# syshin1014/wssdl_bus

Measured on AMD Instinct MI355X. Metric: images/sec (train step, 600x1000), higher is better.
Workload: dtype f32; 1 GPU; resnet50_joint_b8; backbone=ResNet-50, image=600x1000, images_per_gpu=8, supervised_per_gpu=4, weak_per_gpu=4, mode=joint, parallelism=image-parallel dp1, RCCL grad all-reduce, sampling_rng=device, fused_rpn_softmax=True, padded_rois=False, miopen_find=True, miopen_find_db=wssdl_bus_amd/miopen_db (HIP.3_5_0_20250912-42-1199-g2584e35062), miopen_searched=True

## Files before the change

wssdl_bus_amd/csrc/plumbing/rowbn.hip:

```cpp
#include <hip/hip_runtime.h>
#include <stdint.h>

#define PLUMB_API extern "C" __attribute__((visibility("default")))

namespace {

constexpr int BLOCK = 256;
constexpr int MAX_PARTIAL_BLOCKS = 1024;

typedef float float4v __attribute__((ext_vector_type(4)));

template <int MASK>
__device__ __forceinline__ unsigned mask_roi(long long r, int div) {
    return MASK == 2 ? (unsigned)r % (unsigned)div : (unsigned)r / (unsigned)div;
}

__device__ __forceinline__ float bn_affine(float x, float sc, float sh) { return __builtin_fmaf(x, sc, sh); }
__device__ __forceinline__ float bn_dx(float ka, float u, float k0, float k1, float x) {
    return __builtin_fmaf(-k1, x, __builtin_fmaf(ka, u, -k0));
}
__device__ __forceinline__ void acc_rows2(double &s, double &q, float v0, float w0, float v1, float w1) {
    s += (double)v0 + (double)v1;
    q += (double)v0 * (double)w0 + (double)v1 * (double)w1;
}
// ... 4 lines not shown

struct Slab {
    int C4, L, RS, lc, lr;
    long long r0, r1;
    __device__ __forceinline__ Slab(long long M, int C, long long rows_per_block) {
        C4 = C >> 2;
        L = C4 < BLOCK ? C4 : BLOCK;
        RS = BLOCK / L;
        lc = threadIdx.x % L;
        lr = threadIdx.x / L;
        r0 = (long long)blockIdx.x * rows_per_block;
        r1 = r0 + rows_per_block < M ? r0 + rows_per_block : M;
    }
};

__device__ __forceinline__ void slab_reduce(const Slab &b, int C, int c4, const double (&s)[4], const double (&q)[4],
                                            double (*red)[8], double *__restrict__ out) {
    const int t = threadIdx.x;
    __syncthreads();
#pragma unroll
    for (int j = 0; j < 4; ++j) { red[t][j] = s[j]; red[t][4 + j] = q[j]; }
    __syncthreads();
    if (b.lr == 0) {
#pragma unroll
        for (int j = 0; j < 4; ++j) {
            double ss = 0.0, qq = 0.0;
            for (int k = 0; k < b.RS; ++k) { ss += red[k * b.L + b.lc][j]; qq += red[k * b.L + b.lc][4 + j]; }
            out[c4 * 4 + j] = ss;
            out[C + c4 * 4 + j] = qq;
        }
    }
}

template <int MODE, bool RELU, int MASK>
__global__ __launch_bounds__(BLOCK) void rowbn_partial_kernel(
    const float *__restrict__ x, const float *__restrict__ dy, const float *__restrict__ scale,
    const float *__restrict__ shift, long long M, int C, long long rows_per_block,
    double *__restrict__ partial, const float *__restrict__ mask, int per) {
    __shared__ double red[BLOCK][8];
    const Slab b(M, C, rows_per_block);
    const int C4 = b.C4, L = b.L, RS = b.RS, lc = b.lc, lr = b.lr;
    const long long r0 = b.r0, r1 = b.r1;
    double *out = partial + (size_t)blockIdx.x * 2 * C;
    for (int cc = 0; cc * L < C4; ++cc) {
        const int c4 = cc * L + lc;
        double s[4] = {0, 0, 0, 0}, q[4] = {0, 0, 0, 0};
        float4v sc = {0, 0, 0, 0}, sh = {0, 0, 0, 0};
        if (MODE == 1 && RELU) {
            sc = reinterpret_cast<const float4v *>(scale)[c4];
            sh = reinterpret_cast<const float4v *>(shift)[c4];
        }
        if (lr < RS) {
            long long r = r0 + lr;
            for (; r + RS < r1; r += 2 * RS) {
                bool live0 = true, live1 = true;
                if (MASK) {
                    live0 = mask[mask_roi<MASK>(r, per)] != 0.0f;
                    live1 = mask[mask_roi<MASK>(r + RS, per)] != 0.0f;
                    if (!live0 && !live1) continue;
                }
                const float4v zero4 = {0, 0, 0, 0};
                const float4v a0 = live0 ? reinterpret_cast<const float4v *>(x + (size_t)r * C)[c4] : zero4;
                const float4v a1 = live1 ? reinterpret_cast<const float4v *>(x + (size_t)(r + RS) * C)[c4] : zero4;
                float4v g0, g1;
                if (MODE == 1) {
                    g0 = live0 ? reinterpret_cast<const float4v *>(dy + (size_t)r * C)[c4] : zero4;
                    g1 = live1 ? reinterpret_cast<const float4v *>(dy + (size_t)(r + RS) * C)[c4] : zero4;
                }
#pragma unroll
                for (int j = 0; j < 4; ++j) {
                    if (MODE == 0) {
                        acc_rows2(s[j], q[j], a0[j], a0[j], a1[j], a1[j]);
                    } else {
                        float u0 = g0[j], u1 = g1[j];
                        if (RELU) {
                            if (!(bn_affine(a0[j], sc[j], sh[j]) > 0.0f)) u0 = 0.0f;
                            if (!(bn_affine(a1[j], sc[j], sh[j]) > 0.0f)) u1 = 0.0f;
                        }
                        if (MASK) {
                            if (!live0) u0 = 0.0f;
                            if (!live1) u1 = 0.0f;
                        }
                        acc_rows2(s[j], q[j], u0, a0[j], u1, a1[j]);
                    }
                }
            }
            for (; r < r1; r += RS) {
                if (MASK && mask[mask_roi<MASK>(r, per)] == 0.0f) continue;
                const float4v a0 = reinterpret_cast<const float4v *>(x + (size_t)r * C)[c4];
                float4v g0;
                if (MODE == 1) g0 = reinterpret_cast<const float4v *>(dy + (size_t)r * C)[c4];
#pragma unroll
                for (int j = 0; j < 4; ++j) {
                    if (MODE == 0) {
                        acc_row(s[j], q[j], a0[j], a0[j]);
                    } else {
                        float u0 = g0[j];
                        if (RELU && !(bn_affine(a0[j], sc[j], sh[j]) > 0.0f)) u0 = 0.0f;
                        acc_row(s[j], q[j], u0, a0[j]);
                    }
                }
            }
        }
        slab_reduce(b, C, c4, s, q, red, out);
    }
}

constexpr int FIN_COLS = 16, FIN_GROUPS = 64;

__device__ __forceinline__ void finish_reduce(const double *__restrict__ partial, int nblocks, int C,
                                              int c, int grp, double (*red)[FIN_COLS][2], double &s,
                                              double &q) {
    double ss = 0.0, qq = 0.0;
    if (c < C)
        for (int b = grp; b < nblocks; b += FIN_GROUPS) {
            ss += partial[(size_t)b * 2 * C + c];
            qq += partial[(size_t)b * 2 * C + C + c];
        }
    red[grp][threadIdx.x % FIN_COLS][0] = ss;
    red[grp][threadIdx.x % FIN_COLS][1] = qq;
    __syncthreads();
    s = 0.0;
    q = 0.0;
    if (grp == 0)
// ... 64 lines not shown
    dweight[c] = (float)sum_g_xhat;
    dbias[c] = (float)sg;
    coef[c] = (float)a;
    coef[C + c] = (float)k0;
    coef[2 * C + c] = (float)k1;
}

template <bool RELU, int MASK>
__global__ __launch_bounds__(BLOCK) void rowbn_apply_fwd_kernel(
    const float *__restrict__ x, const float *__restrict__ scale, const float *__restrict__ shift,
    long long total4, int C4, float *__restrict__ y, const float *__restrict__ mask, int per) {
    for (long long i = (long long)blockIdx.x * BLOCK + threadIdx.x; i < total4;
         i += (long long)gridDim.x * BLOCK) {
        const int c4 = (int)(i % C4);
        if (MASK && mask[mask_roi<MASK>(i / C4, per)] == 0.0f) {
            const float4v zero4 = {0, 0, 0, 0};
            reinterpret_cast<float4v *>(y)[i] = zero4;
            continue;
        }
        const float4v a = reinterpret_cast<const float4v *>(x)[i];
        const float4v sc = reinterpret_cast<const float4v *>(scale)[c4];
        const float4v sh = reinterpret_cast<const float4v *>(shift)[c4];
        float4v o;
#pragma unroll
        for (int j = 0; j < 4; ++j) {
            float v = bn_affine(a[j], sc[j], sh[j]);
            if (RELU) v = v > 0.0f ? v : 0.0f;
            o[j] = v;
        }
        reinterpret_cast<float4v *>(y)[i] = o;
    }
}

template <bool RELU, int MASK>
__global__ __launch_bounds__(BLOCK) void rowbn_apply_bwd_kernel(
    const float *__restrict__ x, const float *__restrict__ dy, const float *__restrict__ scale,
    const float *__restrict__ shift, const float *__restrict__ coef, long long total4, int C4,
    float *__restrict__ dx, const float *__restrict__ mask, int per) {
    const int C = C4 * 4;
    for (long long i = (long long)blockIdx.x * BLOCK + threadIdx.x; i < total4;
         i += (long long)gridDim.x * BLOCK) {
        const int c4 = (int)(i % C4);
        if (MASK && mask[mask_roi<MASK>(i / C4, per)] == 0.0f) {
            const float4v zero4 = {0, 0, 0, 0};
            reinterpret_cast<float4v *>(dx)[i] = zero4;
            continue;
        }
        const float4v a = reinterpret_cast<const float4v *>(x)[i];
        const float4v g = reinterpret_cast<const float4v *>(dy)[i];
        const float4v ka = reinterpret_cast<const float4v *>(coef)[c4];
        const float4v k0 = reinterpret_cast<const float4v *>(coef + C)[c4];
        const float4v k1 = reinterpret_cast<const float4v *>(coef + 2 * C)[c4];
        float4v sc = {0, 0, 0, 0}, sh = {0, 0, 0, 0};
        if (RELU) {
            sc = reinterpret_cast<const float4v *>(scale)[c4];
            sh = reinterpret_cast<const float4v *>(shift)[c4];
        }
        float4v o;
#pragma unroll
        for (int j = 0; j < 4; ++j) {
            float u = g[j];
            if (RELU && !(bn_affine(a[j], sc[j], sh[j]) > 0.0f)) u = 0.0f;
            o[j] = bn_dx(ka[j], u, k0[j], k1[j], a[j]);
        }
        reinterpret_cast<float4v *>(dx)[i] = o;
    }
}


template <int MASK>
__device__ __forceinline__ bool row_live(const float *__restrict__ mask, long long r, int div) {
    return MASK ? mask[mask_roi<MASK>(r, div)] != 0.0f : true;
}

__device__ __forceinline__ float4v load4(const float *__restrict__ p, long long r, int C, int c4, bool on) {
    const float4v zero4 = {0, 0, 0, 0};
    return on ? reinterpret_cast<const float4v *>(p + (size_t)r * C)[c4] : zero4;
}

template <bool DUAL, int MASK>
__global__ __launch_bounds__(BLOCK) void rowbn_join_fwd_kernel(
    const float *__restrict__ x3, const float *__restrict__ sc3, const float *__restrict__ sh3,
// ... 286 lines not shown
                         workspace, workspace_bytes, stream);
}

PLUMB_API int wsplumb_rowbn_backward_masked(const float *x, const float *dy, long long M, int C,
                                            const float *weight, const float *mean, const float *rstd,
                                            const float *scale, const float *shift, int relu,
                                            const float *mask, int n_rois, int per, float *dx,
                                            float *dweight, float *dbias, float *coef, void *workspace,
                                            size_t workspace_bytes, void *stream) {
    if (!mask) return 1;
    return backward_impl(x, dy, M, C, weight, mean, rstd, scale, shift, relu, dx, dweight, dbias, coef, mask, n_rois, per,
                         workspace, workspace_bytes, stream);
}

PLUMB_API int wsplumb_rowbn_forward_masked_pm(const float *x, long long M, int C, const float *weight,
                                              const float *bias, float eps, int relu, const float *mask,
                                              int n_rois, int per, float *y, float *mean, float *var,
                                              float *rstd, float *scale, float *shift, float *count,
                                              void *workspace, size_t workspace_bytes, void *stream) {
    if (!mask || !count) return 1;
    return forward_impl(x, M, C, weight, bias, eps, relu, y, mean, var, rstd, scale, shift, mask, n_rois, per, count,
                        workspace, workspace_bytes, stream, true);
}

PLUMB_API int wsplumb_rowbn_backward_masked_pm(const float *x, const float *dy, long long M, int C,
                                               const float *weight, const float *mean, const float *rstd,
                                               const float *scale, const float *shift, int relu,
                                               const float *mask, int n_rois, int per, float *dx,
                                               float *dweight, float *dbias, float *coef, void *workspace,
                                               size_t workspace_bytes, void *stream) {
    if (!mask) return 1;
    return backward_impl(x, dy, M, C, weight, mean, rstd, scale, shift, relu, dx, dweight, dbias, coef, mask, n_rois, per,
                         workspace, workspace_bytes, stream, true);
}


PLUMB_API size_t wsplumb_rowbn_join_workspace_bytes(long long M, int C) {
    return 2 * wsplumb_rowbn_workspace_bytes(M, C);
}

namespace {

struct JoinGeom {
    hipStream_t st;
    int nb, mode, div;
    long long rpb, total4;
    double *p0, *p1;
};

inline int join_geom(long long M, int C, const float *mask, int n_rois, int per, void *workspace,
                     size_t workspace_bytes, void *stream, JoinGeom &g) {
    if (!shape_ok(M, C) || workspace_bytes < wsplumb_rowbn_join_workspace_bytes(M, C)) return 1;
    if (mask && (per < 1 || n_rois < 1 || (long long)n_rois * per != M || M > 0x7fffffffLL)) return 1;
    g.st = static_cast<hipStream_t>(stream);
    g.nb = partial_blocks(M, C);
    g.rpb = (M + g.nb - 1) / g.nb;
    g.total4 = M * (C / 4);
    g.mode = mask ? 2 : 0;
    g.div = mask ? n_rois : 1;
    g.p0 = static_cast<double *>(workspace);
    g.p1 = g.p0 + (size_t)g.nb * 2 * C;
    return 0;
}

inline void join_stats(const JoinGeom &g, const float *x, long long M, int C, const float *weight, const float *bias,
                       float eps, float *stats, const float *mask, int n_rois, int per, float *count) {
// ... 99 lines not shown
```

wssdl_bus_amd/csrc/plumbing/taps.hip:

```cpp
#include <hip/hip_runtime.h>
#include <stdint.h>

#define PLUMB_API extern "C" __attribute__((visibility("default")))

namespace {

constexpr int TAB_NCLS = 0, TAB_H = 1, TAB_W = 2, TAB_OH = 3, TAB_OW = 4, TAB_S = 5, TAB_PT = 6, TAB_PL = 7,
              TAB_UNITS = 8, TAB_WUNITS = 9;
constexpr int TAB_CLS = 16, CLS_STRIDE = 24, MAX_CLS = 9;
constexpr int C_NPOS = 0, C_NTAPS = 1, C_SLOT = 2, C_CUM = 3, C_WCUM = 4,
              C_TAPS = 6,
              C_TAPIDX = 15;
constexpr int MAX_POS = 64;
constexpr int TAB_SLOTPOS = TAB_CLS + CLS_STRIDE * MAX_CLS;
constexpr int TAB_POSSLOT = TAB_SLOTPOS + MAX_POS;
constexpr int TAB_SLOTCLS = TAB_POSSLOT + MAX_POS;
constexpr int TAB_INTS = TAB_SLOTCLS + MAX_POS;

typedef float float4v __attribute__((ext_vector_type(4)));

__device__ __forceinline__ const int *cls_of(const int *T, int k) { return T + TAB_CLS + CLS_STRIDE * k; }

template <int F>
__device__ __forceinline__ int find_class(const int *__restrict__ T, unsigned q) {
    const int n = T[TAB_NCLS];
    int k = 0;
    while (k + 1 < n && (unsigned)cls_of(T, k + 1)[F] <= q) ++k;
    return k;
}

__global__ __launch_bounds__(256) void tap_gather_kernel(const float *__restrict__ x, const int *__restrict__ T,
                                                        int in_pm, unsigned R, unsigned C4, unsigned total4,
                                                        float *__restrict__ cols) {
    const int H = T[TAB_H], W = T[TAB_W], OW = T[TAB_OW], S = T[TAB_S], PT = T[TAB_PT], PL = T[TAB_PL];
    const unsigned unit4 = R * C4;
    for (unsigned i = blockIdx.x * 256u + threadIdx.x; i < total4; i += gridDim.x * 256u) {
        const int k = find_class<C_CUM>(T, i / unit4);
        const int *cl = cls_of(T, k);
        const unsigned ntaps = cl[C_NTAPS];
        const unsigned local = i - (unsigned)cl[C_CUM] * unit4;
        const unsigned c4 = local % C4, t = local / C4;
        const unsigned tl = t % ntaps, row = t / ntaps;
        const unsigned roi = row % R, p = row / R;
        const int pos = T[TAB_SLOTPOS + cl[C_SLOT] + p];
        const int tap = cl[C_TAPS + tl];
        const int y = (pos / OW) * S + tap / 3 - PT, xx = (pos % OW) * S + tap % 3 - PL;
        float4v v = {0.f, 0.f, 0.f, 0.f};
        if (y >= 0 && y < H && xx >= 0 && xx < W) {
            const size_t src = in_pm ? (size_t)T[TAB_POSSLOT + y * W + xx] * R + roi
                                     : ((size_t)roi * H + y) * W + xx;
            v = reinterpret_cast<const float4v *>(x)[src * C4 + c4];
        }
        reinterpret_cast<float4v *>(cols)[i] = v;
    }
}

__global__ __launch_bounds__(256) void tap_col2im_kernel(const float *__restrict__ dcols, const int *__restrict__ T,
                                                        int in_pm, unsigned R, unsigned C4, unsigned total4,
                                                        float *__restrict__ dx) {
    const int H = T[TAB_H], W = T[TAB_W], OH = T[TAB_OH], OW = T[TAB_OW], S = T[TAB_S], PT = T[TAB_PT],
              PL = T[TAB_PL];
    const unsigned unit4 = R * C4;
    for (unsigned i = blockIdx.x * 256u + threadIdx.x; i < total4; i += gridDim.x * 256u) {
        const unsigned c4 = i % C4, row = i / C4;
        unsigned roi;
        int y, xx;
        if (in_pm) {
            roi = row % R;
            const int pos = T[TAB_SLOTPOS + row / R];
            y = pos / W;
            xx = pos % W;
        } else {
            xx = (int)(row % (unsigned)W);
            const unsigned t = row / (unsigned)W;
            y = (int)(t % (unsigned)H);
            roi = t / (unsigned)H;
        }
        float4v acc = {0.f, 0.f, 0.f, 0.f};
#pragma unroll
        for (int ky = 0; ky < 3; ++ky) {
            const int ny = y + PT - ky;
            if (ny < 0 || ny % S != 0) continue;
            const int oy = ny / S;
            if (oy >= OH) continue;
#pragma unroll
            for (int kx = 0; kx < 3; ++kx) {
                const int nx = xx + PL - kx;
                if (nx < 0 || nx % S != 0) continue;
                const int ox = nx / S;
                if (ox >= OW) continue;
                const int slot = T[TAB_POSSLOT + oy * OW + ox];
                const int *cl = cls_of(T, T[TAB_SLOTCLS + slot]);
                const int tl = cl[C_TAPIDX + ky * 3 + kx];
                if (tl < 0) continue;
                const size_t u = (size_t)cl[C_CUM] * unit4 +
                                 (((size_t)(slot - cl[C_SLOT]) * R + roi) * cl[C_NTAPS] + tl) * C4 + c4;
                acc += reinterpret_cast<const float4v *>(dcols)[u];
            }
        }
        reinterpret_cast<float4v *>(dx)[i] = acc;
    }
}

__global__ __launch_bounds__(256) void tap_weight_gather_kernel(const float *__restrict__ w, const int *__restrict__ T,
                                                               unsigned CO, unsigned C4, unsigned total4,
                                                               float *__restrict__ wp) {
    const unsigned unit4 = CO * C4;
    for (unsigned i = blockIdx.x * 256u + threadIdx.x; i < total4; i += gridDim.x * 256u) {
        const int k = find_class<C_WCUM>(T, i / unit4);
        const int *cl = cls_of(T, k);
        const unsigned ntaps = cl[C_NTAPS];
        const unsigned local = i - (unsigned)cl[C_WCUM] * unit4;
        const unsigned c4 = local % C4, t = local / C4;
        const unsigned tl = t % ntaps, o = t / ntaps;
        reinterpret_cast<float4v *>(wp)[i] =
            reinterpret_cast<const float4v *>(w)[((size_t)o * 9 + cl[C_TAPS + tl]) * C4 + c4];
    }
}

__global__ __launch_bounds__(256) void tap_weight_scatter_kernel(const float *__restrict__ dwp, const int *__restrict__ T,
                                                                unsigned CO, unsigned C4, unsigned total4,
                                                                float *__restrict__ dw) {
    const int n = T[TAB_NCLS];
    const unsigned unit4 = CO * C4;
    for (unsigned i = blockIdx.x * 256u + threadIdx.x; i < total4; i += gridDim.x * 256u) {
        const unsigned c4 = i % C4, t = i / C4;
        const unsigned tap = t % 9u, o = t / 9u;
        float4v acc = {0.f, 0.f, 0.f, 0.f};
        for (int k = 0; k < n; ++k) {
            const int *cl = cls_of(T, k);
            const int tl = cl[C_TAPIDX + tap];
            if (tl < 0) continue;
            acc += reinterpret_cast<const float4v *>(dwp)[(size_t)cl[C_WCUM] * unit4 +
                                                           ((size_t)o * cl[C_NTAPS] + tl) * C4 + c4];
        }
        reinterpret_cast<float4v *>(dw)[i] = acc;
    }
}

inline int grid_for(unsigned total4) {
    unsigned b = (total4 + 255u) / 256u;
    return (int)(b < 262144u ? b : 262144u);
}

inline bool dims_ok(long long R, int C, long long total4) {
    return R >= 1 && C >= 4 && !(C & 3) && total4 >= 1 && total4 <= 0x7fffffffLL;
}

}

PLUMB_API int wsplumb_tap_table_ints() { return TAB_INTS; }

PLUMB_API int wsplumb_tap_gather(const float *x, long long R, int C, const int *tab, const int *hnum, int in_pm,
                                 float *cols, void *stream) {
    const long long total4 = (long long)hnum[TAB_UNITS] * R * (C / 4);
    if (R < 1 || C < 4 || (C & 3)) return 1;
    if (!dims_ok(R, C, total4) || (long long)hnum[TAB_H] * hnum[TAB_W] * R * (C / 4) > 0x7fffffffLL) return 2;
    hipLaunchKernelGGL(tap_gather_kernel, dim3(grid_for((unsigned)total4)), dim3(256), 0,
                       static_cast<hipStream_t>(stream), x, tab, in_pm, (unsigned)R, (unsigned)(C / 4),
                       (unsigned)total4, cols);
    return hipGetLastError() == hipSuccess ? 0 : 3;
}

PLUMB_API int wsplumb_tap_col2im(const float *dcols, long long R, int C, const int *tab, const int *hnum, int in_pm,
                                 float *dx, void *stream) {
    const long long total4 = (long long)hnum[TAB_H] * hnum[TAB_W] * R * (C / 4);
    if (R < 1 || C < 4 || (C & 3)) return 1;
    if (!dims_ok(R, C, total4) || (long long)hnum[TAB_UNITS] * R * (C / 4) > 0x7fffffffLL) return 2;
    hipLaunchKernelGGL(tap_col2im_kernel, dim3(grid_for((unsigned)total4)), dim3(256), 0,
                       static_cast<hipStream_t>(stream), dcols, tab, in_pm, (unsigned)R, (unsigned)(C / 4),
                       (unsigned)total4, dx);
    return hipGetLastError() == hipSuccess ? 0 : 3;
}

PLUMB_API int wsplumb_tap_weight_gather(const float *w, int CO, int C, const int *tab, const int *hnum, float *wp,
                                        void *stream) {
    const long long total4 = (long long)hnum[TAB_WUNITS] * CO * (C / 4);
    if (CO < 1 || !dims_ok(CO, C, total4) || 9LL * CO * (C / 4) > 0x7fffffffLL) return 1;
    hipLaunchKernelGGL(tap_weight_gather_kernel, dim3(grid_for((unsigned)total4)), dim3(256), 0,
                       static_cast<hipStream_t>(stream), w, tab, (unsigned)CO, (unsigned)(C / 4), (unsigned)total4, wp);
    return hipGetLastError() == hipSuccess ? 0 : 3;
}

PLUMB_API int wsplumb_tap_weight_scatter(const float *dwp, int CO, int C, const int *tab, const int *hnum, float *dw,
                                         void *stream) {
    const long long total4 = 9LL * CO * (C / 4);
    if (CO < 1 || !dims_ok(CO, C, total4) || (long long)hnum[TAB_WUNITS] * CO * (C / 4) > 0x7fffffffLL) return 1;
    hipLaunchKernelGGL(tap_weight_scatter_kernel, dim3(grid_for((unsigned)total4)), dim3(256), 0,
                       static_cast<hipStream_t>(stream), dwp, tab, (unsigned)CO, (unsigned)(C / 4), (unsigned)total4, dw);
    return hipGetLastError() == hipSuccess ? 0 : 3;
}
```

wssdl_bus_amd/networks/_plumbing.py:

```python
import ctypes
import os
import warnings

import torch

_HERE = os.path.dirname(os.path.dirname(os.path.abspath(__file__)))
LIB_PATH = os.path.join(_HERE, "libwssdl_plumbing_hip.so")
_lib = None
_warned = [False]

_vp, _i, _ll, _f, _sz = ctypes.c_void_p, ctypes.c_int, ctypes.c_longlong, ctypes.c_float, ctypes.c_size_t


def lib():
    global _lib
    if _lib is None:
        if not os.path.exists(LIB_PATH):
            if not _warned[0]:
                _warned[0] = True
                warnings.warn("%s not built: the per-RoI head uses stock PyTorch batch-norm ops "
                              "(python -m wssdl_bus_amd.build builds it)" % LIB_PATH)
            return None
        L = ctypes.CDLL(LIB_PATH)
        L.wsplumb_rowbn_workspace_bytes.restype = _sz
        L.wsplumb_rowbn_workspace_bytes.argtypes = [_ll, _i]
        L.wsplumb_rowbn_supported.restype = _i
        L.wsplumb_rowbn_supported.argtypes = [_ll, _i]
        L.wsplumb_rowbn_forward.restype = _i
        L.wsplumb_rowbn_forward.argtypes = [_vp, _ll, _i, _vp, _vp, _f, _i, _vp, _vp, _vp, _vp, _vp, _vp,
                                            _vp, _sz, _vp]
        L.wsplumb_rowbn_apply.restype = _i
        L.wsplumb_rowbn_apply.argtypes = [_vp, _ll, _i, _vp, _vp, _i, _vp, _vp]
        L.wsplumb_rowbn_backward.restype = _i
        L.wsplumb_rowbn_backward.argtypes = [_vp, _vp, _ll, _i, _vp, _vp, _vp, _vp, _vp, _i, _vp, _vp, _vp,
                                             _vp, _vp, _sz, _vp]
        L.wsplumb_rowbn_forward_masked.restype = _i
        L.wsplumb_rowbn_forward_masked.argtypes = [_vp, _ll, _i, _vp, _vp, _f, _i, _vp, _i, _i, _vp, _vp, _vp, _vp,
                                                   _vp, _vp, _vp, _vp, _sz, _vp]
        L.wsplumb_rowbn_backward_masked.restype = _i
        L.wsplumb_rowbn_backward_masked.argtypes = [_vp, _vp, _ll, _i, _vp, _vp, _vp, _vp, _vp, _i, _vp, _i, _i,
                                                    _vp, _vp, _vp, _vp, _vp, _sz, _vp]
        for name in ("wsplumb_rowbn_forward_masked_pm", "wsplumb_rowbn_backward_masked_pm"):
            base = getattr(L, name[:-3])
            getattr(L, name).restype, getattr(L, name).argtypes = base.restype, base.argtypes
        L.wsplumb_rowbn_join_workspace_bytes.restype = _sz
        L.wsplumb_rowbn_join_workspace_bytes.argtypes = [_ll, _i]
        L.wsplumb_rowbn_join_forward.restype = _i
        L.wsplumb_rowbn_join_forward.argtypes = [_vp, _vp, _ll, _i, _vp, _vp, _f, _vp, _vp, _f, _vp, _vp, _f, _vp, _i, _i,
                                                 _vp, _vp, _vp, _vp, _vp, _vp, _vp, _sz, _vp]
        L.wsplumb_rowbn_join_backward.restype = _i
        L.wsplumb_rowbn_join_backward.argtypes = [_vp] * 5 + [_ll, _i] + [_vp] * 7 + [_i, _i] + [_vp] * 8 + [_sz, _vp]
        L.wsplumb_tap_table_ints.restype = _i
        L.wsplumb_tap_table_ints.argtypes = []
        for name in ("wsplumb_tap_gather", "wsplumb_tap_col2im"):
            f = getattr(L, name)
            f.restype = _i
            f.argtypes = [_vp, _ll, _i, _vp, _vp, _i, _vp, _vp]
        for name in ("wsplumb_tap_weight_gather", "wsplumb_tap_weight_scatter"):
            f = getattr(L, name)
            f.restype = _i
            f.argtypes = [_vp, _i, _i, _vp, _vp, _vp, _vp]
        for name in ("wsplumb_im2col3x3", "wsplumb_col2im3x3"):
            f = getattr(L, name)
            f.restype = _i
            f.argtypes = [_vp, _ll, _i, _i, _i, _i, _i, _i, _i, _i, _vp, _vp]
        _lib = L
    return _lib


def _p(t):
    return ctypes.c_void_p(t.data_ptr())


def _stream():
    return ctypes.c_void_p(torch.cuda.current_stream().cuda_stream)


# ... 38 lines not shown


def rowbn_apply(x, scale, shift, relu):
    L = lib()
    M, C = x.shape
    y = torch.empty_like(x)
    with torch.cuda.device(x.device):
        rc = L.wsplumb_rowbn_apply(_p(x), M, C, _p(scale), _p(shift), int(relu), _p(y), _stream())
    if rc:
        raise RuntimeError("wsplumb_rowbn_apply failed (%d)" % rc)
    return y


def rowbn_backward(x, dy, weight, stats, relu, mask=None, pos_major=False):
    L = lib()
    M, C = x.shape
    dev = x.device
    dx = torch.empty_like(x)
    dwb = torch.empty((2, C), dtype=torch.float32, device=dev)
    coef = torch.empty((3, C), dtype=torch.float32, device=dev)
    with torch.cuda.device(dev):
        ws, n = _workspace(L, M, C, dev)
        if mask is None:
            rc = L.wsplumb_rowbn_backward(_p(x), _p(dy), M, C, _p(weight), _p(stats[0]), _p(stats[2]),
                                          _p(stats[3]), _p(stats[4]), int(relu), _p(dx), _p(dwb[0]),
                                          _p(dwb[1]), _p(coef), _p(ws), n, _stream())
        else:
            n_rois = mask.shape[0]
            fn = L.wsplumb_rowbn_backward_masked_pm if pos_major else L.wsplumb_rowbn_backward_masked
            rc = fn(_p(x), _p(dy), M, C, _p(weight), _p(stats[0]), _p(stats[2]), _p(stats[3]), _p(stats[4]), int(relu),
                    _p(mask), n_rois, M // n_rois, _p(dx), _p(dwb[0]), _p(dwb[1]), _p(coef), _p(ws), n, _stream())
    if rc:
        raise RuntimeError("wsplumb_rowbn_backward failed (%d)" % rc)
    return dx, dwb[0], dwb[1]


def join_usable(x):
    if os.environ.get("WSSDL_HEAD_UNFUSED_JOIN"):
        return False
    return usable(x)


def _pn(t):
    return _p(t) if t is not None else None


def rowbn_join_forward(x3, bn3, other, bns, bnn, mask=None):
    L = lib()
    M, C = x3.shape
    dev = x3.device
    assert other.shape == x3.shape and other.is_contiguous() and other.dtype == torch.float32
    out, y = torch.empty_like(x3), torch.empty_like(x3)
    stats = torch.empty((3, 5, C), dtype=torch.float32, device=dev)
    count, n_rois = None, 0
    if mask is not None:
        n_rois = mask.shape[0]
        assert M % n_rois == 0 and mask.dtype == torch.float32 and mask.is_contiguous()
        count = torch.empty((1,), dtype=torch.float32, device=dev)
    ws_, bs_, es_ = bns if bns is not None else (None, None, 0.0)
    with torch.cuda.device(dev):
        n = L.wsplumb_rowbn_join_workspace_bytes(M, C)
        ws = torch.empty((n,), dtype=torch.uint8, device=dev)
        rc = L.wsplumb_rowbn_join_forward(_p(x3), _p(other), M, C, _p(bn3[0]), _p(bn3[1]), float(bn3[2]), _pn(ws_),
                                          _pn(bs_), float(es_), _p(bnn[0]), _p(bnn[1]), float(bnn[2]), _pn(mask), n_rois,
                                          M // n_rois if n_rois else 1, _p(out), _p(y), _p(stats[0]),
                                          _p(stats[1]) if bns is not None else None, _p(stats[2]), _pn(count), _p(ws), n,
# ... 115 lines not shown
    def _table(self):
        import numpy as np
        T = np.full(_TAB_INTS, -1, np.int32)
        T[:10] = [len(self.classes), self.h, self.w, self.oh, self.ow, self.s, self.pt, self.pl, self.units,
                  self.wunits]
        for k, (taps, pos) in enumerate(self.classes[:_MAX_CLS]):
            b = _TAB_CLS + _CLS_STRIDE * k
            T[b:b + 5] = [len(pos), len(taps), self.slot_base[k], self.cum[k], self.wcum[k]]
            T[b + 6:b + 6 + len(taps)] = taps
            for i, t in enumerate(taps):
                T[b + 15 + t] = i
        for sl, (y, x) in enumerate(self.slots[:_MAX_POS]):
            T[_TAB_SLOTPOS + sl] = y * self.ow + x
            T[_TAB_POSSLOT + y * self.ow + x] = sl
            T[_TAB_SLOTCLS + sl] = next(k for k in range(len(self.classes))
                                        if self.slot_base[k] <= sl < self.slot_base[k] + len(self.classes[k][1]))
        return T

    def device_table(self, dev):
        t = self._dev.get(dev)
        if t is None:
            t = self._dev[dev] = torch.from_numpy(self.table).to(dev)
        return t

    def subsample_index(self, w_in, s, dev):
        key = ("sub", w_in, s, dev)
        t = self._dev.get(key)
        if t is None:
            t = self._dev[key] = torch.tensor([y * s * w_in + x * s for y, x in self.slots],
                                              dtype=torch.long, device=dev)
        return t


_PLANS = {}


def tap_plan(h, w, s):
    p = _PLANS.get((h, w, s))
    if p is None:
        p = _PLANS[(h, w, s)] = TapPlan(h, w, s)
    return p


def taps_usable(x):
    if os.environ.get("WSSDL_HEAD_DENSE_3X3"):
        return False
    return im2col_usable(x) and x.shape[0] >= TAPS_MIN_ROIS


def _tap_call(name, *args):
    rc = getattr(lib(), name)(*args, _stream())
    if rc:
        raise RuntimeError("%s failed (%d)" % (name, rc))


def tap_gather(x, plan, in_pm, R):
    C = x.shape[-1]
    cols = torch.empty((plan.units * R * C,), dtype=torch.float32, device=x.device)
    with torch.cuda.device(x.device):
        _tap_call("wsplumb_tap_gather", _p(x), R, C, _p(plan.device_table(x.device)), plan.hnum, int(in_pm), _p(cols))
    return cols


def tap_col2im(dcols, plan, in_pm, R, C):
    shape = (plan.h * plan.w * R, C) if in_pm else (R, plan.h, plan.w, C)
    dx = torch.empty(shape, dtype=torch.float32, device=dcols.device)
# ... 95 lines not shown
```

wssdl_bus_amd/networks/roi_head.py:

```python
import torch
import torch.nn as nn
import torch.nn.functional as F

from . import _plumbing
from .backbones import RESNET_DEFS, _same_pad


class _RowBatchNormFn(torch.autograd.Function):

    @staticmethod
    def forward(ctx, x, weight, bias, eps):
        var, mean = torch.var_mean(x, dim=0, unbiased=False)
        rstd = torch.rsqrt(var + eps)
        scale = rstd * weight
        y = torch.addcmul(bias - mean * scale, x, scale)
        ctx.save_for_backward(x, mean, rstd, weight)
        ctx.mark_non_differentiable(mean, var)
        return y, mean, var

    @staticmethod
    def backward(ctx, dy, _dmean, _dvar):
        x, mean, rstd, weight = ctx.saved_tensors
        m = x.shape[0]
        sum_dy = dy.sum(0)
# ... 29 lines not shown
            x, weight, stats, roi_mask = ctx.saved_tensors
        else:
            (x, weight, stats), roi_mask = ctx.saved_tensors, None
        dx, dw, db = _plumbing.rowbn_backward(x, dy.contiguous(), weight, stats, ctx.relu, roi_mask, ctx.pos_major)
        return dx, dw, db, None, None, None, None


class _JoinFn(torch.autograd.Function):

    @staticmethod
    def forward(ctx, x3, other, w3, b3, ws, bs, wn, bn, eps3, eps_s, eps_n, roi_mask):
        dual = ws is not None
        out, y, st3, sts, stn, count = _plumbing.rowbn_join_forward(
            x3, (w3, b3, eps3), other, (ws, bs, eps_s) if dual else None, (wn, bn, eps_n), roi_mask)
        ctx.dual, ctx.masked = dual, roi_mask is not None
        ctx.save_for_backward(x3, other if dual else None, out, w3, ws, wn, st3, sts, stn, roi_mask)
        if count is None:
            count = stn[0, :1]
        ctx.mark_non_differentiable(st3, sts, stn, count)
        ctx.set_materialize_grads(False)
        return out, y, st3, sts, stn, count

    @staticmethod
    def backward(ctx, dres, dy, *_):
        x3, xs, out, w3, ws, wn, st3, sts, stn, roi_mask = ctx.saved_tensors
        if dy is None:
            dy = torch.zeros_like(out)
        g, dx3, dxs, dwbn, dwb3, dwbs = _plumbing.rowbn_join_backward(
            out, dy.contiguous(), dres.contiguous() if dres is not None else None, x3, xs, wn, stn, w3, st3, ws, sts,
            roi_mask)
        if ctx.dual:
            return dx3, dxs, dwb3[0], dwb3[1], dwbs[0], dwbs[1], dwbn[0], dwbn[1], None, None, None, None
        return dx3, g, dwb3[0], dwb3[1], None, None, dwbn[0], dwbn[1], None, None, None, None


_ROI_MASK = None


def set_roi_mask(mask):
    global _ROI_MASK
    _ROI_MASK = mask


def _masked_row_batch_norm(x, weight, bias, eps, relu, roi_mask, pos_major=False):
    M = x.shape[0]
    per = M // roi_mask.shape[0]
    m = (roi_mask.repeat(per) if pos_major else roi_mask.repeat_interleave(per)).unsqueeze(1)
    n = (roi_mask.sum() * per).clamp_min(1.0)
    mean = (x * m).sum(0) / n
    d = (x - mean) * m
    var = (d * d).sum(0) / n
    y = d * (torch.rsqrt(var + eps) * weight) + bias
    if relu:
        y = F.relu(y)
    return y * m, mean.detach(), var.detach(), n


class RowBatchNorm(nn.Module):

    def __init__(self, num_features, eps=1e-3, momentum=0.01):
        super().__init__()
        self.eps, self.momentum = eps, momentum
        self.weight = nn.Parameter(torch.ones(num_features))
        self.bias = nn.Parameter(torch.zeros(num_features))
        self.register_buffer("running_mean", torch.zeros(num_features))
        self.register_buffer("running_var", torch.ones(num_features))
# ... 86 lines not shown
    return x.view(r, h * w, c).transpose(0, 1).index_select(0, idx).reshape(-1, c)


def _bn_rows(bn, x, relu=False):
    r, h, w, c = x.shape
    return bn(x.reshape(-1, c), relu=relu).view(r, h, w, c)


class BottleneckNHWC(nn.Module):
    expansion = 4

    def __init__(self, c_i, c_o, s, preact, norm):
        super().__init__()
        self.preact = preact
        self.pre_bn = RowBatchNorm(c_i) if (preact != "no_preact" and norm == "BN") else None
        self.conv1 = ConvNHWC(c_i, c_o, 1, 1, norm)
        self.conv2 = ConvNHWC(c_o, c_o, 3, s, norm)
        self.conv3 = ConvNHWC(c_o, c_o * 4, 1, 1, norm, relu=False)
        self.short = ConvNHWC(c_i, c_o * 4, 1, s, norm, relu=False) if c_i != c_o * 4 else None

    def forward(self, x):
        ori = x
        if self.preact != "no_preact":
            y = _bn_rows(self.pre_bn, x, relu=True) if self.pre_bn is not None else F.relu(x)
            if self.preact == "both_preact":
                ori = y
            x = y
        x = self.conv3(self.conv2(self.conv1(x)))
        return x + (self.short(ori) if self.short is not None else ori)

    def forward_pm(self, x, plans, R, pre=None, nxt=None):
        pm = x.dim() == 2
        ori = x
        if self.preact != "no_preact":
            y = pre if pre is not None else _pre_act(self.pre_bn, x, pm)
            if self.preact == "both_preact":
                ori = y
            x = y
        s = self.conv2.s
        plan = plans[s]
        if not pm:
            x = self.conv1(x)
        else:
            x = self.conv1.forward_pm(x, plan, R)
        x = self.conv3.forward_pm(self.conv2.forward_pm(x, plan, R), plan, R, act=False)
        return _join_pm(self.conv3, x, self.short, ori, plan, s, R, nxt)


class BasicBlockNHWC(nn.Module):
    expansion = 1

    def __init__(self, c_i, c_o, s, preact, norm):
        super().__init__()
        self.preact = preact
        self.pre_bn = RowBatchNorm(c_i) if (preact != "no_preact" and norm == "BN") else None
        self.conv1 = ConvNHWC(c_i, c_o, 3, s, norm)
        self.conv2 = ConvNHWC(c_o, c_o, 3, 1, norm, relu=False)
        self.short = ConvNHWC(c_i, c_o, 1, s, norm, relu=False) if c_i != c_o else None

    def forward(self, x):
        ori = x
        if self.preact != "no_preact":
            y = _bn_rows(self.pre_bn, x, relu=True) if self.pre_bn is not None else F.relu(x)
            if self.preact == "both_preact":
                ori = y
            x = y
        x = self.conv2(self.conv1(x))
        return x + (self.short(ori) if self.short is not None else ori)

    def forward_pm(self, x, plans, R, pre=None, nxt=None):
        pm = x.dim() == 2
        ori = x
        if self.preact != "no_preact":
            y = pre if pre is not None else _pre_act(self.pre_bn, x, pm)
            if self.preact == "both_preact":
                ori = y
            x = y
        s = self.conv1.s
        plan = plans[s]
        x = self.conv2.forward_pm(self.conv1.forward_pm(x, plan, R), plans[1], R, act=False)
        return _join_pm(self.conv2, x, self.short, ori, plan, s, R, nxt)


def _join_pm(last, x3, short, ori, plan, s, R, nxt):
    if short is not None:
        xs = short.forward_pm(ori, plan, R, act=False)
    else:
        xs = ori if ori.dim() == 2 else _pm_rows(ori, plan, s)
    bns = [last.bn, nxt] + ([short.bn] if short is not None else [])
    mask = _ROI_MASK
    if (nxt is None or any(b is None or not b.training for b in bns) or last.relu or not _plumbing.join_usable(x3)
            or (mask is not None and x3.shape[0] % mask.shape[0] != 0)):
        return last._act(x3, pos_major=True) + (short._act(xs, pos_major=True) if short is not None else xs), None
    b3, bs = last.bn, short.bn if short is not None else None
    out, y, st3, sts, stn, n = _JoinFn.apply(
        x3, xs.contiguous(), b3.weight, b3.bias, bs.weight if bs is not None else None,
        bs.bias if bs is not None else None, nxt.weight, nxt.bias, b3.eps, bs.eps if bs is not None else 0.0, nxt.eps,
        mask)
    n = n[0] if mask is not None else x3.shape[0]
    b3._track(st3[0], st3[1], n)
    if bs is not None:
        bs._track(sts[0], sts[1], n)
    nxt._track(stn[0], stn[1], n)
    return out, y


def _pre_act(bn, x, pm):
    if not pm:
        return _bn_rows(bn, x, relu=True) if bn is not None else F.relu(x)
    return bn(x, relu=True, pos_major=True) if bn is not None else F.relu(x)


class ResNetHeadNHWC(nn.Module):

    def __init__(self, depth, norm="BN"):
        super().__init__()
        defs, block = RESNET_DEFS[depth]
        blk = BottleneckNHWC if block.expansion == 4 else BasicBlockNHWC
        e = blk.expansion
        blocks = [blk(256 * e, 512, 2, "both_preact", norm)]
        for _ in range(1, defs[3]):
            blocks.append(blk(512 * e, 512, 1, "default", norm))
        self.group3 = nn.Sequential(*blocks)
        self.norm = RowBatchNorm(512 * e) if norm == "BN" else None
        self.out_features = 512 * e

    def forward(self, x):
        plans = self._tap_plans(x)
        if plans is not None:
            return self._forward_pm(x, plans)
        x = self.group3(x)
        x = _bn_rows(self.norm, x, relu=True) if self.norm is not None else F.relu(x)
        return x.mean(dim=(1, 2))

    @staticmethod
    def _tap_plans(x):
        if not _plumbing.taps_usable(x):
            return None
        p2 = _plumbing.tap_plan(x.shape[1], x.shape[2], 2)
# ... 16 lines not shown
```

Measured before the change: 52.78 images/s.

## Fuse head entry BN backward with shortcut grad scatter; restructure tap gather/col2im grids

Adds a fused entry path for the first ROI-head bottleneck: the pre-activation BN forward also produces the subsampled position-major rows for the shortcut, and its backward folds the shortcut gradient (scattered through a position-to-slot table) into the BN backward kernels. This removes a separate scatter/add and extra passes over the gradient. Separately, the tap gather and col2im kernels are rewritten to use a 2D grid (ROI chunks by tap unit or position), hoisting table lookups and address math per block and coalescing channel loads. The extra indirect load per dy element and the new grid limits are the main risks.

```diff
diff --git a/wssdl_bus_amd/csrc/plumbing/rowbn.hip b/wssdl_bus_amd/csrc/plumbing/rowbn.hip
--- a/wssdl_bus_amd/csrc/plumbing/rowbn.hip
+++ b/wssdl_bus_amd/csrc/plumbing/rowbn.hip
@@ -60,11 +60,29 @@
     }
 }
 
-template <int MODE, bool RELU, int MASK>
+struct EntryGrad {
+    const float *dys;
+    const int *possel;
+    int per, R;
+};
+
+template <bool ENTRY>
+__device__ __forceinline__ float4v load_dy(const float *__restrict__ dy, const EntryGrad &e, long long r, int C, int c4) {
+    const float4v g = reinterpret_cast<const float4v *>(dy + (size_t)r * C)[c4];
+    if (!ENTRY) return g;
+    const unsigned roi = (unsigned)r / (unsigned)e.per, p = (unsigned)r - roi * (unsigned)e.per;
+    const int slot = e.possel[p];
+    const float4v zero4 = {0, 0, 0, 0};
+    float4v d = zero4;
+    if (slot >= 0) d = reinterpret_cast<const float4v *>(e.dys + ((size_t)slot * e.R + roi) * C)[c4] + zero4;
+    return g + d;
+}
+
+template <int MODE, bool RELU, int MASK, bool ENTRY = false>
 __global__ __launch_bounds__(BLOCK) void rowbn_partial_kernel(
     const float *__restrict__ x, const float *__restrict__ dy, const float *__restrict__ scale,
     const float *__restrict__ shift, long long M, int C, long long rows_per_block,
-    double *__restrict__ partial, const float *__restrict__ mask, int per) {
+    double *__restrict__ partial, const float *__restrict__ mask, int per, EntryGrad eg = EntryGrad()) {
     __shared__ double red[BLOCK][8];
     const Slab b(M, C, rows_per_block);
     const int C4 = b.C4, L = b.L, RS = b.RS, lc = b.lc, lr = b.lr;
@@ -92,8 +110,8 @@
                 const float4v a1 = live1 ? reinterpret_cast<const float4v *>(x + (size_t)(r + RS) * C)[c4] : zero4;
                 float4v g0, g1;
                 if (MODE == 1) {
-                    g0 = live0 ? reinterpret_cast<const float4v *>(dy + (size_t)r * C)[c4] : zero4;
-                    g1 = live1 ? reinterpret_cast<const float4v *>(dy + (size_t)(r + RS) * C)[c4] : zero4;
+                    g0 = live0 ? load_dy<ENTRY>(dy, eg, r, C, c4) : zero4;
+                    g1 = live1 ? load_dy<ENTRY>(dy, eg, r + RS, C, c4) : zero4;
                 }
 #pragma unroll
                 for (int j = 0; j < 4; ++j) {
@@ -117,7 +135,7 @@
                 if (MASK && mask[mask_roi<MASK>(r, per)] == 0.0f) continue;
                 const float4v a0 = reinterpret_cast<const float4v *>(x + (size_t)r * C)[c4];
                 float4v g0;
-                if (MODE == 1) g0 = reinterpret_cast<const float4v *>(dy + (size_t)r * C)[c4];
+                if (MODE == 1) g0 = load_dy<ENTRY>(dy, eg, r, C, c4);
 #pragma unroll
                 for (int j = 0; j < 4; ++j) {
                     if (MODE == 0) {
@@ -248,11 +266,11 @@
     }
 }
 
-template <bool RELU, int MASK>
+template <bool RELU, int MASK, bool ENTRY = false>
 __global__ __launch_bounds__(BLOCK) void rowbn_apply_bwd_kernel(
     const float *__restrict__ x, const float *__restrict__ dy, const float *__restrict__ scale,
     const float *__restrict__ shift, const float *__restrict__ coef, long long total4, int C4,
-    float *__restrict__ dx, const float *__restrict__ mask, int per) {
+    float *__restrict__ dx, const float *__restrict__ mask, int per, EntryGrad eg = EntryGrad()) {
     const int C = C4 * 4;
     for (long long i = (long long)blockIdx.x * BLOCK + threadIdx.x; i < total4;
          i += (long long)gridDim.x * BLOCK) {
@@ -263,7 +281,7 @@
             continue;
         }
         const float4v a = reinterpret_cast<const float4v *>(x)[i];
-        const float4v g = reinterpret_cast<const float4v *>(dy)[i];
+        const float4v g = ENTRY ? load_dy<true>(dy, eg, i / C4, C, c4) : reinterpret_cast<const float4v *>(dy)[i];
         const float4v ka = reinterpret_cast<const float4v *>(coef)[c4];
         const float4v k0 = reinterpret_cast<const float4v *>(coef + C)[c4];
         const float4v k1 = reinterpret_cast<const float4v *>(coef + 2 * C)[c4];
@@ -616,6 +634,39 @@
     if (!mask) return 1;
     return backward_impl(x, dy, M, C, weight, mean, rstd, scale, shift, relu, dx, dweight, dbias, coef, mask, n_rois, per,
                          workspace, workspace_bytes, stream, true);
+}
+
+PLUMB_API int wsplumb_rowbn_backward_entry(const float *x, const float *dy, const float *dys, const int *possel,
+                                           int n_slots, long long M, int C, const float *weight, const float *mean,
+                                           const float *rstd, const float *scale, const float *shift,
+                                           const float *mask, int n_rois, int per, float *dx, float *dweight,
+                                           float *dbias, float *coef, void *workspace, size_t workspace_bytes,
+                                           void *stream) {
+    if (!shape_ok(M, C) || workspace_bytes < wsplumb_rowbn_workspace_bytes(M, C)) return 1;
+    if (!dys || !possel || per < 1 || n_rois < 1 || n_slots < 1 || n_slots > per ||
+        (long long)n_rois * per != M || M > 0x7fffffffLL)
+        return 1;
+    hipStream_t st = static_cast<hipStream_t>(stream);
+    const int nb = partial_blocks(M, C);
+    const long long rpb = (M + nb - 1) / nb;
+    double *partial = static_cast<double *>(workspace);
+    const EntryGrad eg = {dys, possel, per, n_rois};
+    if (mask)
+        hipLaunchKernelGGL((rowbn_partial_kernel<1, true, 1, true>), dim3(nb), dim3(BLOCK), 0, st, x, dy, scale, shift, M,
+                           C, rpb, partial, mask, per, eg);
+    else
+        hipLaunchKernelGGL((rowbn_partial_kernel<1, true, 0, true>), dim3(nb), dim3(BLOCK), 0, st, x, dy, scale, shift, M,
+                           C, rpb, partial, mask, 1, eg);
+    hipLaunchKernelGGL(rowbn_bwd_finish_kernel, dim3((C + FIN_COLS - 1) / FIN_COLS), dim3(FIN_COLS * FIN_GROUPS), 0, st,
+                       partial, nb, C, M, weight, mean, rstd, dweight, dbias, coef, mask, n_rois, per);
+    const long long total4 = M * (C / 4);
+    if (mask)
+        hipLaunchKernelGGL((rowbn_apply_bwd_kernel<true, 1, true>), dim3(apply_grid(total4)), dim3(BLOCK), 0, st, x, dy,
+                           scale, shift, coef, total4, C / 4, dx, mask, per, eg);
+    else
+        hipLaunchKernelGGL((rowbn_apply_bwd_kernel<true, 0, true>), dim3(apply_grid(total4)), dim3(BLOCK), 0, st, x, dy,
+                           scale, shift, coef, total4, C / 4, dx, mask, 1, eg);
+    return hipGetLastError() == hipSuccess ? 0 : 3;
 }
 
 
diff --git a/wssdl_bus_amd/csrc/plumbing/taps.hip b/wssdl_bus_amd/csrc/plumbing/taps.hip
--- a/wssdl_bus_amd/csrc/plumbing/taps.hip
+++ b/wssdl_bus_amd/csrc/plumbing/taps.hip
@@ -29,76 +29,93 @@
     return k;
 }
 
+struct RoiWalk {
+    unsigned L, RS, lc, lr, roi0, roi1;
+    __device__ __forceinline__ RoiWalk(unsigned R, unsigned C4, unsigned chunk) {
+        L = (C4 <= 256u && 256u % C4 == 0u) ? C4 : 256u;
+        RS = 256u / L;
+        lc = threadIdx.x % L;
+        lr = threadIdx.x / L;
+        roi0 = blockIdx.x * chunk;
+        roi1 = roi0 + chunk < R ? roi0 + chunk : R;
+    }
+};
+
+constexpr unsigned GATHER_CHUNK = 32, COL2IM_CHUNK = 16;
+
 __global__ __launch_bounds__(256) void tap_gather_kernel(const float *__restrict__ x, const int *__restrict__ T,
-                                                        int in_pm, unsigned R, unsigned C4, unsigned total4,
+                                                        int in_pm, unsigned R, unsigned C4,
                                                         float *__restrict__ cols) {
     const int H = T[TAB_H], W = T[TAB_W], OW = T[TAB_OW], S = T[TAB_S], PT = T[TAB_PT], PL = T[TAB_PL];
-    const unsigned unit4 = R * C4;
-    for (unsigned i = blockIdx.x * 256u + threadIdx.x; i < total4; i += gridDim.x * 256u) {
-        const int k = find_class<C_CUM>(T, i / unit4);
-        const int *cl = cls_of(T, k);
-        const unsigned ntaps = cl[C_NTAPS];
-        const unsigned local = i - (unsigned)cl[C_CUM] * unit4;
-        const unsigned c4 = local % C4, t = local / C4;
-        const unsigned tl = t % ntaps, row = t / ntaps;
-        const unsigned roi = row % R, p = row / R;
-        const int pos = T[TAB_SLOTPOS + cl[C_SLOT] + p];
-        const int tap = cl[C_TAPS + tl];
-        const int y = (pos / OW) * S + tap / 3 - PT, xx = (pos % OW) * S + tap % 3 - PL;
-        float4v v = {0.f, 0.f, 0.f, 0.f};
-        if (y >= 0 && y < H && xx >= 0 && xx < W) {
-            const size_t src = in_pm ? (size_t)T[TAB_POSSLOT + y * W + xx] * R + roi
-                                     : ((size_t)roi * H + y) * W + xx;
-            v = reinterpret_cast<const float4v *>(x)[src * C4 + c4];
-        }
-        reinterpret_cast<float4v *>(cols)[i] = v;
+    const unsigned q = blockIdx.y;
+    const int *cl = cls_of(T, find_class<C_CUM>(T, q));
+    const unsigned ntaps = cl[C_NTAPS], local = q - (unsigned)cl[C_CUM];
+    const unsigned p = local / ntaps, tl = local - p * ntaps;
+    const int pos = T[TAB_SLOTPOS + cl[C_SLOT] + p];
+    const int tap = cl[C_TAPS + tl];
+    const int y = (pos / OW) * S + tap / 3 - PT, xx = (pos % OW) * S + tap % 3 - PL;
+    const bool inside = y >= 0 && y < H && xx >= 0 && xx < W;
+    const unsigned sbase = !inside ? 0u : in_pm ? (unsigned)T[TAB_POSSLOT + y * W + xx] * R * C4 : (unsigned)(y * W + xx) * C4;
+    const unsigned sstride = in_pm ? C4 : (unsigned)(H * W) * C4;
+    const unsigned dstride = ntaps * C4;
+    const unsigned dbase = (unsigned)cl[C_CUM] * R * C4 + p * R * dstride + tl * C4;
+    const float4v *__restrict__ src = reinterpret_cast<const float4v *>(x) + sbase;
+    float4v *__restrict__ dst = reinterpret_cast<float4v *>(cols) + dbase;
+    const RoiWalk w(R, C4, GATHER_CHUNK);
+    const float4v zero4 = {0.f, 0.f, 0.f, 0.f};
+    for (unsigned c4 = w.lc; c4 < C4; c4 += w.L) {
+        unsigned roi = w.roi0 + w.lr;
+        for (; roi + 3u * w.RS < w.roi1; roi += 4u * w.RS) {
+            float4v v[4];
+#pragma unroll
+            for (int k = 0; k < 4; ++k) v[k] = inside ? src[(roi + k * w.RS) * sstride + c4] : zero4;
+#pragma unroll
+            for (int k = 0; k < 4; ++k) dst[(roi + k * w.RS) * dstride + c4] = v[k];
+        }
+        for (; roi < w.roi1; roi += w.RS) dst[roi * dstride + c4] = inside ? src[roi * sstride + c4] : zero4;
     }
 }
 
 __global__ __launch_bounds__(256) void tap_col2im_kernel(const float *__restrict__ dcols, const int *__restrict__ T,
-                                                        int in_pm, unsigned R, unsigned C4, unsigned total4,
+                                                        int in_pm, unsigned R, unsigned C4,
                                                         float *__restrict__ dx) {
     const int H = T[TAB_H], W = T[TAB_W], OH = T[TAB_OH], OW = T[TAB_OW], S = T[TAB_S], PT = T[TAB_PT],
               PL = T[TAB_PL];
-    const unsigned unit4 = R * C4;
-    for (unsigned i = blockIdx.x * 256u + threadIdx.x; i < total4; i += gridDim.x * 256u) {
-        const unsigned c4 = i % C4, row = i / C4;
-        unsigned roi;
-        int y, xx;
-        if (in_pm) {
-            roi = row % R;
-            const int pos = T[TAB_SLOTPOS + row / R];
-            y = pos / W;
-            xx = pos % W;
-        } else {
-            xx = (int)(row % (unsigned)W);
-            const unsigned t = row / (unsigned)W;
-            y = (int)(t % (unsigned)H);
-            roi = t / (unsigned)H;
-        }
-        float4v acc = {0.f, 0.f, 0.f, 0.f};
-#pragma unroll
-        for (int ky = 0; ky < 3; ++ky) {
-            const int ny = y + PT - ky;
-            if (ny < 0 || ny % S != 0) continue;
-            const int oy = ny / S;
-            if (oy >= OH) continue;
-#pragma unroll
-            for (int kx = 0; kx < 3; ++kx) {
-                const int nx = xx + PL - kx;
-                if (nx < 0 || nx % S != 0) continue;
-                const int ox = nx / S;
-                if (ox >= OW) continue;
-                const int slot = T[TAB_POSSLOT + oy * OW + ox];
-                const int *cl = cls_of(T, T[TAB_SLOTCLS + slot]);
-                const int tl = cl[C_TAPIDX + ky * 3 + kx];
-                if (tl < 0) continue;
-                const size_t u = (size_t)cl[C_CUM] * unit4 +
-                                 (((size_t)(slot - cl[C_SLOT]) * R + roi) * cl[C_NTAPS] + tl) * C4 + c4;
-                acc += reinterpret_cast<const float4v *>(dcols)[u];
-            }
-        }
-        reinterpret_cast<float4v *>(dx)[i] = acc;
+    const int pos = in_pm ? T[TAB_SLOTPOS + blockIdx.y] : (int)blockIdx.y;
+    const int y = pos / W, xx = pos % W;
+    unsigned base[9], stride[9], valid = 0;
+#pragma unroll
+    for (int ky = 0; ky < 3; ++ky) {
+#pragma unroll
+        for (int kx = 0; kx < 3; ++kx) {
+            const int j = ky * 3 + kx;
+            base[j] = stride[j] = 0;
+            const int ny = y + PT - ky, nx = xx + PL - kx;
+            if (ny < 0 || ny % S != 0 || nx < 0 || nx % S != 0) continue;
+            const int oy = ny / S, ox = nx / S;
+            if (oy >= OH || ox >= OW) continue;
+            const int slot = T[TAB_POSSLOT + oy * OW + ox];
+            const int *cl = cls_of(T, T[TAB_SLOTCLS + slot]);
+            const int tl = cl[C_TAPIDX + j];
+            if (tl < 0) continue;
+            stride[j] = (unsigned)cl[C_NTAPS] * C4;
+            base[j] = (unsigned)cl[C_CUM] * R * C4 + (unsigned)(slot - cl[C_SLOT]) * R * stride[j] + (unsigned)tl * C4;
+            valid |= 1u << j;
+        }
+    }
+    const float4v *__restrict__ src = reinterpret_cast<const float4v *>(dcols);
+    const unsigned dbase = in_pm ? blockIdx.y * R * C4 : (unsigned)pos * C4;
+    const unsigned dstride = in_pm ? C4 : (unsigned)(H * W) * C4;
+    float4v *__restrict__ dst = reinterpret_cast<float4v *>(dx) + dbase;
+    const RoiWalk w(R, C4, COL2IM_CHUNK);
+    for (unsigned c4 = w.lc; c4 < C4; c4 += w.L) {
+        for (unsigned roi = w.roi0 + w.lr; roi < w.roi1; roi += w.RS) {
+            float4v acc = {0.f, 0.f, 0.f, 0.f};
+#pragma unroll
+            for (int j = 0; j < 9; ++j)
+                if (valid & (1u << j)) acc += src[base[j] + roi * stride[j] + c4];
+            dst[roi * dstride + c4] = acc;
+        }
     }
 }
 
@@ -143,6 +160,8 @@
     return (int)(b < 262144u ? b : 262144u);
 }
 
+inline unsigned roi_chunks(long long R, unsigned chunk) { return (unsigned)((R + chunk - 1) / chunk); }
+
 inline bool dims_ok(long long R, int C, long long total4) {
     return R >= 1 && C >= 4 && !(C & 3) && total4 >= 1 && total4 <= 0x7fffffffLL;
 }
@@ -156,9 +175,9 @@
     const long long total4 = (long long)hnum[TAB_UNITS] * R * (C / 4);
     if (R < 1 || C < 4 || (C & 3)) return 1;
     if (!dims_ok(R, C, total4) || (long long)hnum[TAB_H] * hnum[TAB_W] * R * (C / 4) > 0x7fffffffLL) return 2;
-    hipLaunchKernelGGL(tap_gather_kernel, dim3(grid_for((unsigned)total4)), dim3(256), 0,
-                       static_cast<hipStream_t>(stream), x, tab, in_pm, (unsigned)R, (unsigned)(C / 4),
-                       (unsigned)total4, cols);
+    if (hnum[TAB_UNITS] < 1 || hnum[TAB_UNITS] > 65535) return 1;
+    hipLaunchKernelGGL(tap_gather_kernel, dim3(roi_chunks(R, GATHER_CHUNK), hnum[TAB_UNITS]), dim3(256), 0,
+                       static_cast<hipStream_t>(stream), x, tab, in_pm, (unsigned)R, (unsigned)(C / 4), cols);
     return hipGetLastError() == hipSuccess ? 0 : 3;
 }
 
@@ -167,9 +186,9 @@
     const long long total4 = (long long)hnum[TAB_H] * hnum[TAB_W] * R * (C / 4);
     if (R < 1 || C < 4 || (C & 3)) return 1;
     if (!dims_ok(R, C, total4) || (long long)hnum[TAB_UNITS] * R * (C / 4) > 0x7fffffffLL) return 2;
-    hipLaunchKernelGGL(tap_col2im_kernel, dim3(grid_for((unsigned)total4)), dim3(256), 0,
-                       static_cast<hipStream_t>(stream), dcols, tab, in_pm, (unsigned)R, (unsigned)(C / 4),
-                       (unsigned)total4, dx);
+    if (hnum[TAB_H] * hnum[TAB_W] < 1 || hnum[TAB_H] * hnum[TAB_W] > MAX_POS) return 1;
+    hipLaunchKernelGGL(tap_col2im_kernel, dim3(roi_chunks(R, COL2IM_CHUNK), hnum[TAB_H] * hnum[TAB_W]), dim3(256), 0,
+                       static_cast<hipStream_t>(stream), dcols, tab, in_pm, (unsigned)R, (unsigned)(C / 4), dx);
     return hipGetLastError() == hipSuccess ? 0 : 3;
 }
 
diff --git a/wssdl_bus_amd/networks/_plumbing.py b/wssdl_bus_amd/networks/_plumbing.py
--- a/wssdl_bus_amd/networks/_plumbing.py
+++ b/wssdl_bus_amd/networks/_plumbing.py
@@ -43,6 +43,8 @@
         for name in ("wsplumb_rowbn_forward_masked_pm", "wsplumb_rowbn_backward_masked_pm"):
             base = getattr(L, name[:-3])
             getattr(L, name).restype, getattr(L, name).argtypes = base.restype, base.argtypes
+        L.wsplumb_rowbn_backward_entry.restype = _i
+        L.wsplumb_rowbn_backward_entry.argtypes = [_vp] * 4 + [_i, _ll, _i] + [_vp] * 6 + [_i, _i] + [_vp] * 5 + [_sz, _vp]
         L.wsplumb_rowbn_join_workspace_bytes.restype = _sz
         L.wsplumb_rowbn_join_workspace_bytes.argtypes = [_ll, _i]
         L.wsplumb_rowbn_join_forward.restype = _i
@@ -147,6 +149,34 @@
                     _p(mask), n_rois, M // n_rois, _p(dx), _p(dwb[0]), _p(dwb[1]), _p(coef), _p(ws), n, _stream())
     if rc:
         raise RuntimeError("wsplumb_rowbn_backward failed (%d)" % rc)
+    return dx, dwb[0], dwb[1]
+
+
+def entry_usable(x):
+    if os.environ.get("WSSDL_HEAD_UNFUSED_ENTRY"):
+        return False
+    return usable(x) and x.shape[0] < 2 ** 31
+
+
+def rowbn_backward_entry(x, dy, dys, possel, n_slots, weight, stats, mask=None):
+    L = lib()
+    M, C = x.shape
+    dev = x.device
+    per = possel.shape[0]
+    n_rois = M // per
+    assert M == n_rois * per and dy.shape == x.shape and dys.shape == (n_slots * n_rois, C)
+    assert dy.is_contiguous() and dys.is_contiguous() and possel.dtype == torch.int32 and possel.is_contiguous()
+    assert mask is None or (mask.shape[0] == n_rois and mask.dtype == torch.float32 and mask.is_contiguous())
+    dx = torch.empty_like(x)
+    dwb = torch.empty((2, C), dtype=torch.float32, device=dev)
+    coef = torch.empty((3, C), dtype=torch.float32, device=dev)
+    with torch.cuda.device(dev):
+        ws, n = _workspace(L, M, C, dev)
+        rc = L.wsplumb_rowbn_backward_entry(_p(x), _p(dy), _p(dys), _p(possel), n_slots, M, C, _p(weight), _p(stats[0]),
+                                            _p(stats[2]), _p(stats[3]), _p(stats[4]), _pn(mask), n_rois, per, _p(dx),
+                                            _p(dwb[0]), _p(dwb[1]), _p(coef), _p(ws), n, _stream())
+    if rc:
+        raise RuntimeError("wsplumb_rowbn_backward_entry failed (%d)" % rc)
     return dx, dwb[0], dwb[1]
 
 
@@ -328,6 +358,17 @@
         return t
 
 
+    def subsample_slots(self, h_in, w_in, s, dev):
+        key = ("subinv", h_in, w_in, s, dev)
+        t = self._dev.get(key)
+        if t is None:
+            inv = [-1] * (h_in * w_in)
+            for sl, (y, x) in enumerate(self.slots):
+                inv[y * s * w_in + x * s] = sl
+            t = self._dev[key] = torch.tensor(inv, dtype=torch.int32, device=dev)
+        return t
+
+
 _PLANS = {}
 
 
diff --git a/wssdl_bus_amd/networks/roi_head.py b/wssdl_bus_amd/networks/roi_head.py
--- a/wssdl_bus_amd/networks/roi_head.py
+++ b/wssdl_bus_amd/networks/roi_head.py
@@ -85,6 +85,32 @@
         if ctx.dual:
             return dx3, dxs, dwb3[0], dwb3[1], dwbs[0], dwbs[1], dwbn[0], dwbn[1], None, None, None, None
         return dx3, g, dwb3[0], dwb3[1], None, None, dwbn[0], dwbn[1], None, None, None, None
+
+
+class _EntryNormFn(torch.autograd.Function):
+
+    @staticmethod
+    def forward(ctx, x, weight, bias, eps, roi_mask, plan, s, hw):
+        y, stats, count = _plumbing.rowbn_forward(x, weight, bias, eps, True, roi_mask, False)
+        h, w = hw
+        r = x.shape[0] // (h * w)
+        ys = _pm_rows(y.view(r, h, w, -1), plan, s)
+        ctx.save_for_backward(x, weight, stats, roi_mask)
+        ctx.geom = (plan, s, h, w)
+        if count is None:
+            count = stats[0, :1]
+        mean, var = stats[0], stats[1]
+        ctx.mark_non_differentiable(mean, var, count)
+        return y, ys, mean, var, count
+
+    @staticmethod
+    def backward(ctx, dy, dys, *_):
+        x, weight, stats, roi_mask = ctx.saved_tensors
+        plan, s, h, w = ctx.geom
+        dx, dw, db = _plumbing.rowbn_backward_entry(x, dy.contiguous(), dys.contiguous(),
+                                                    plan.subsample_slots(h, w, s, x.device), len(plan.slots), weight,
+                                                    stats, roi_mask)
+        return dx, dw, db, None, None, None, None, None
 
 
 _ROI_MASK = None
@@ -237,19 +263,30 @@
     def forward_pm(self, x, plans, R, pre=None, nxt=None):
         pm = x.dim() == 2
         ori = x
-        if self.preact != "no_preact":
+        s = self.conv2.s
+        plan = plans[s]
+        if self._entry_fused(x, pre):
+            x, ori = _entry_pre_act(self.pre_bn, x, plan, s)
+        elif self.preact != "no_preact":
             y = pre if pre is not None else _pre_act(self.pre_bn, x, pm)
             if self.preact == "both_preact":
                 ori = y
             x = y
-        s = self.conv2.s
-        plan = plans[s]
         if not pm:
             x = self.conv1(x)
         else:
             x = self.conv1.forward_pm(x, plan, R)
         x = self.conv3.forward_pm(self.conv2.forward_pm(x, plan, R), plan, R, act=False)
         return _join_pm(self.conv3, x, self.short, ori, plan, s, R, nxt)
+
+
+    def _entry_fused(self, x, pre):
+        bn, mask = self.pre_bn, _ROI_MASK
+        if x.dim() != 4 or pre is not None or self.preact != "both_preact" or self.short is None or bn is None:
+            return False
+        rows = x.reshape(-1, x.shape[3])
+        return (bn.training and torch.is_grad_enabled() and _plumbing.entry_usable(rows)
+                and (mask is None or rows.shape[0] % mask.shape[0] == 0))
 
 
 class BasicBlockNHWC(nn.Module):
@@ -310,6 +347,13 @@
     return out, y
 
 
+def _entry_pre_act(bn, x, plan, s):
+    r, h, w, c = x.shape
+    y, ys, mean, var, n = _EntryNormFn.apply(x.reshape(-1, c), bn.weight, bn.bias, bn.eps, _ROI_MASK, plan, s, (h, w))
+    bn._track(mean, var, n[0] if _ROI_MASK is not None else r * h * w)
+    return y.view(r, h, w, c), ys
+
+
 def _pre_act(bn, x, pm):
     if not pm:
         return _bn_rows(bn, x, relu=True) if bn is not None else F.relu(x)
```

After: 54.06 images/s (median of 6 runs). 1.02x the previous value.
